# gpmp-dev/gpmp

Hardware: AMD Instinct MI355X
Metric: fp64 predict+NLL throughput (points/s) and potrf TFLOP/s vs roofline, n=32k (higher is better)
Workload: dtype f64

## Files before the change

gpmp_amd/_lib.py:

```python
from __future__ import annotations

import ctypes
import os
from ctypes import c_char_p, c_double, c_int, c_long, c_size_t, c_void_p

_HERE = os.path.dirname(os.path.abspath(__file__))
LIB_PATH = os.environ.get("GPMP_HIP_LIB") or os.path.join(_HERE, "libgpmp_hip.so")

_lib = None

_P = c_void_p
SIGNATURES = {
    "gpmp_hip_abi_version": (c_int, []),
    "gpmp_last_error": (c_char_p, []),
    "gpmp_profile_begin": (c_int, []),
    "gpmp_profile_begin_kinds": (c_int, [ctypes.c_uint]),
    "gpmp_profile_end": (c_int, [_P]),
    "gpmp_stream_create_reserving_cus": (c_int, [c_int, _P]),
    "gpmp_stream_destroy": (c_int, [_P]),
    "gpmp_stream_release": (c_int, [_P]),
    "gpmp_hint_machine_busy": (c_int, [c_int]),
    "gpmp_matern_gram": (c_int, [_P, _P, c_int, c_int, c_int, c_int, _P, c_int, c_double, c_int, _P, c_long, _P]),
    "gpmp_matern_pairwise": (c_int, [_P, _P, c_int, c_int, c_int, _P, c_int, _P, _P]),
    "gpmp_scaled_distance": (c_int, [_P, _P, c_int, c_int, c_int, _P, _P, c_long, _P]),
    "gpmp_maternp_kernel": (c_int, [_P, c_long, c_int, _P, _P]),
    "gpmp_matern_gram_deriv": (c_int, [_P, c_int, c_int, c_int, _P, c_int, c_int, _P, c_long, _P]),
    "gpmp_dinv_elems": (c_size_t, [c_int]),
    "gpmp_potrf_lower_async": (c_int, [_P, c_int, c_long, _P, _P, _P]),
    "gpmp_potrf_trsm_lower_async": (c_int, [_P, c_int, c_long, _P, _P, _P, c_int, c_long, _P]),
    "gpmp_trsm_lower": (c_int, [_P, c_int, c_long, _P, _P, c_int, c_long, c_int, _P, _P]),
    "gpmp_solve_status": (c_int, [_P, _P]),
    "gpmp_trsm_right_lower": (c_int, [_P, c_int, c_long, _P, _P, c_int, c_long, _P]),
    "gpmp_trtri_diag_blocks": (c_int, [_P, c_int, c_long, _P, _P]),
    "gpmp_trtri_lower": (c_int, [_P, c_int, c_long, _P, _P, c_long, _P]),
    "gpmp_lauum_lower": (c_int, [_P, c_int, c_long, _P, c_long, _P]),
    "gpmp_tril": (c_int, [_P, c_int, c_long, _P]),
    "gpmp_symmetrize_from_lower": (c_int, [_P, c_int, c_long, _P]),
    "gpmp_dgemm": (c_int, [c_int, c_int, c_int, c_int, c_int, c_double, _P, c_long, _P, c_long, c_double, _P, c_long, c_int, _P]),
    "gpmp_coldots": (c_int, [_P, c_int, c_int, c_long, _P, c_int, c_long, _P, c_long, _P, _P]),
    "gpmp_coldots_ws_rows": (c_int, [c_int]),
    "gpmp_device_release": (c_int, []),
    "gpmp_device_state_count": (c_int, []),
    "gpmp_debug_device_table_selftest": (c_int, [c_int, c_int, c_int]),
    "gpmp_jacobi_sweep": (c_int, [_P, c_long, _P, c_long, c_int, c_double, _P, _P]),
# ... 72 lines not shown
```

gpmp_amd/csrc/common.h:

```cpp
#pragma once
#include <hip/hip_runtime.h>
#include <cstdint>
#include <cstdio>
#include <cstring>
#include <atomic>
#include <vector>
#include "../../include/gpmp_hip.h"

namespace gpmp {

typedef double d4 __attribute__((ext_vector_type(4)));
typedef double d2 __attribute__((ext_vector_type(2)));

constexpr int NB = GPMP_NB;
constexpr int OUTER_BLOCKS = 4;

void set_error(const char* fmt, ...);
int hip_fail(hipError_t e, const char* what);

#define GPMP_HIP_TRY(expr)                                   \
  do {                                                       \
    hipError_t e__ = (expr);                                 \
    if (e__ != hipSuccess) return ::gpmp::hip_fail(e__, #expr); \
  } while (0)
// ... 40 lines not shown
};

struct GemmOpts {
  int lower_only = 0;
  int kstart_row = 0;
  int kend_row = 0;
  int kstart_col = 0;
  int kend_col = 0;
  int batch = 1;
  long stride_a = 0, stride_b = 0, stride_c = 0;
  int batch2 = 1;
  long stride2_a = 0, stride2_b = 0, stride2_c = 0;
  int lean = 0;
  int stair_num = 0, stair_den = 0, stair_off = 0, stair_sub = 0;
  int kg_rnum = 0, kg_rden = 0, kg_roff = 0, kg_cnum = 0, kg_cden = 0, kg_coff = 0;
};
int launch_gemm(bool a_kc, bool b_kc, int M, int N, int K, double alpha, const double* A, long lda,
                const double* B, long ldb, double beta, double* C, long ldc, const GemmOpts& o,
                hipStream_t st);

int launch_trsm_leaf_forward(const double* L, long ldl, const double* dinv_leaf, int nb, double* B, long ldb, int ncols,
                             double* G, hipStream_t st);

int launch_potf2_inv(double* A, long lda, int jb, double* dinv, int* info_dev, int offset, hipStream_t st);
int launch_potf2_inv_batch(double* A, long lda, int jb, double* dinv, int* info_dev, int offset, int nprob, long stride_a,
                           long stride_dinv, hipStream_t st);
int launch_trtri_blocks(const double* L, long ldl, int n, double* dinv, hipStream_t st);

constexpr int TRSV_FEW_MAX = 16;
int trsv_few(const double* L, int n, long ldl, const double* dinv, double* B, int m, long ldb, int trans,
             hipStream_t st);

int launch_tril(double* A, int n, long lda, hipStream_t st, int nprob = 1, long prob_stride = 0);
int launch_symmetrize(double* A, int n, long lda, hipStream_t st);
int launch_diag_blocks(double* T, int n, long ldt, const double* dinv, hipStream_t st, int nprob = 1, long prob_stride_t = 0,
                       long prob_stride_dinv = 0);

struct ProblemBatch {
  int nprob = 1;
  long stride_a = 0;
  long stride_dinv = 0;
};
int potrf_blocked_batch(double* A, int n, long lda, double* dinv, int* info_dev, const ProblemBatch& pb, hipStream_t st);
int trtri_doubling_batch(const double* L, int n, long ldl, const double* dinv, double* T, long ldt, const ProblemBatch& pb,
                         long stride_t, hipStream_t st);
int launch_gram_lower_batch(const double* x, long stride_x, const int* ns_dev, int nmax, int d, int p, const double* theta_host,
                            int noise, double diag_add, double* K, long ldk, long stride_k, int nprob, hipStream_t st,
                            const double* pp_dev = nullptr);
int gram_param_block_elems();
void fill_gram_param_block(double* blk, int d, int p, const double* theta, int noise, double diag_add);
int launch_grad_trace_batch(const double* Kinv, long ldk, long stride_kinv, const double* x, long stride_x, const int* ns_dev, int nmax,
// ... 7 lines not shown
```

gpmp_amd/csrc/drivers.hip:

```cpp
#include "matern_device.h"

namespace gpmp {
namespace {

constexpr int QMAX = GPMP_MAX_RANK - 1;
constexpr int QLD = QMAX + 1;

constexpr int SM_LDS = 0, SM_LDP = 1, SM_QUAD = 2, SM_ZKZ = 3, SM_C = 16, SM_TOTAL = 16 + QLD + 8;

__global__ void pack_zp_kernel(const double* __restrict__ z, const double* __restrict__ P, long ldp, int n, int q,
                               double* __restrict__ Y, long ldy) {
  const int i = blockIdx.x * blockDim.x + threadIdx.x;
  if (i >= n) return;
  Y[(long)i * ldy] = z[i];
  for (int a = 0; a < q; ++a) Y[(long)i * ldy + 1 + a] = P[(long)i * ldp + a];
}

__device__ int chol_lds(double (*A)[QLD + 1], int q, int* fail, double* d0) {
  const int t = threadIdx.x, nt = blockDim.x;
  for (int k = t; k < q; k += nt) d0[k] = A[k][k];
  for (int k = 0; k < q; ++k) {
    __syncthreads();
    if (t == 0) {
      const double dkk = A[k][k];
// ... 228 lines not shown


enum : unsigned {
  WS_T = 1u << 0,
  WS_W = 1u << 1,
  WS_X = 1u << 2,
  WS_FG = 1u << 3,
  WS_KIT = 1u << 4,
  WS_MEAN = 1u << 5,
  WS_SCAL = 1u << 6,
  WS_DCOL = 1u << 7,
  WS_PGRAD = 1u << 8,
};
struct DriverLayout {
  long ldn, ldm, ldq;
  size_t K, dinv, T, W, X, F, G, Kit, Gm, PtP, Sinv, small, scal, D, dcol, cd, y, vraw, mu, red, gws, total;
};
DriverLayout driver_layout(int n, int m, int d, int q, unsigned use) {
  DriverLayout l = {};
  l.ldn = pad16(n);
  l.ldm = pad16(m + 2 + q);
  l.ldq = pad16(1 + q);
  const size_t nq = (size_t)n * l.ldq, q1 = (size_t)(q > 0 ? q : 1);
  WsCursor c;
  l.K = c.take((size_t)n * l.ldn);
  l.dinv = c.take(gpmp_dinv_elems(n));
  if (use & WS_T) l.T = c.take((size_t)n * l.ldn);
  if (use & WS_W) l.W = c.take(nq);
  if (use & WS_X) l.X = c.take(nq);
  if (use & WS_FG) { l.F = c.take(nq); l.G = c.take(nq); }
  if (use & WS_KIT) l.Kit = c.take((size_t)n * l.ldm);
// ... 3 lines not shown
    l.Sinv = c.take(q1 * l.ldq);
    l.small = c.take(SM_TOTAL);
  }
  if (use & WS_SCAL) l.scal = c.take(16);
  if (use & WS_KIT) l.D = c.take((size_t)(2 + q) * l.ldm);
  if (use & WS_DCOL) l.dcol = c.take((size_t)n);
  const size_t cd_cols = (use & WS_DCOL) ? (size_t)n : (size_t)(m > 1 + q ? m : 1 + q);
  l.cd = c.take(cd_cols * (size_t)gpmp_coldots_ws_rows(n));
  if (use & WS_PGRAD) {
    l.y = c.take((size_t)n);
    l.vraw = c.take((size_t)m);
    l.mu = c.take(q1 * l.ldm);
    l.red = c.take(gpmp_predict_grad_reduce_ws_elems(n, m, d));
  }
  if (use & WS_FG) l.gws = c.take(gpmp_grad_ws_elems(n, d));
  l.total = c.at;
  return l;
}
constexpr unsigned USE_NLL = WS_W | WS_SCAL;
constexpr unsigned USE_REML = WS_W | WS_MEAN | WS_SCAL;
constexpr unsigned USE_NLL_GRAD = USE_REML | WS_T | WS_X | WS_FG;
constexpr unsigned USE_LOO = USE_REML | WS_T | WS_X | WS_DCOL;
constexpr unsigned USE_PREDICT = WS_KIT;
constexpr unsigned USE_PREDICT_MEAN = WS_KIT | WS_MEAN;
constexpr unsigned USE_PREDICT_GRAD = WS_KIT | WS_MEAN | WS_PGRAD;

struct Cov {
  const double* theta;
  int d, p, noise;
  double sigma2, diag;
// ... 80 lines not shown
}

int predict_solve(const Cov& cov, const DriverLayout& l, const double* xi, const double* zi, const double* Pi, long ldpi,
                  const double* xt, int n, int m, int q, double* ws, int* info_dev, gpmp_stream_t stream) {
  hipStream_t st = as_stream(stream);
  double* K = ws + l.K;
  double* Kit = ws + l.Kit;
  int rc = gpmp_matern_gram(xi, nullptr, n, n, cov.d, cov.p, cov.theta, cov.noise, cov.diag, 1, K, l.ldn, stream);
  if (rc) return rc;
  rc = gpmp_matern_gram(xi, xt, n, m, cov.d, cov.p, cov.theta, cov.noise, 0.0, 0, Kit, l.ldm, stream);
  if (rc) return rc;
  rc = stage_zp(zi, Pi, ldpi, n, q, Kit + m, l.ldm, st);
  if (rc) return rc;
  const int mb = (m + 1 + q) + ((m + 1 + q) & 1);
  if (mb > m + 1 + q) GPMP_HIP_TRY(hipMemset2DAsync(Kit + m + 1 + q, (size_t)l.ldm * sizeof(double), 0, sizeof(double), n, st));
  return gpmp_potrf_trsm_lower_async(K, n, l.ldn, ws + l.dinv, info_dev, Kit, mb, l.ldm, stream);
}
}
}

using namespace gpmp;

extern "C" size_t gpmp_nll_ws_elems(int n) { return n > 0 ? driver_layout(n, 0, 1, 0, USE_NLL).total : 0; }

extern "C" int gpmp_nll_zero_mean(const double* x, const double* z, int n, int d, int p, const double* theta_host,
                                  int noise, double* ws, double* nll_dev, int* info_dev, gpmp_stream_t stream) {
  GPMP_ARG(x != nullptr, 1, "x is NULL");
  GPMP_ARG(z != nullptr, 2, "z is NULL");
  GPMP_ARG(n > 0 && n <= GPMP_MAX_EXTENT, 3, "n outside [1, GPMP_MAX_EXTENT]");
  GPMP_ARG(theta_host != nullptr, 6, "theta is NULL");
  GPMP_ARG(ws != nullptr, 8, "ws is NULL");
// ... 243 lines not shown
```

gpmp_amd/csrc/gemm_f64.hip:

```cpp
#include "common.h"
#include <cstdlib>

namespace gpmp {

int g_machine_busy = 0;

namespace {

constexpr int BM = 128, BN = 128, BK = 16;
constexpr int LDK = 18;
constexpr int LDN = 144;
constexpr int TILE = 2304;
constexpr int NXCD = 8;
typedef unsigned int v4u __attribute__((ext_vector_type(4)));

struct GemmParams {
  const double* A;
  const double* B;
  double* C;
  long lda, ldb, ldc;
  int M, N, K;
  double alpha, beta;
  int lower_only, kstart_row, kend_row, kend_col;
  int kstart_col;
  int tiles_m, tiles_n, ntiles;
  int aligned;
  int lean;
  int batch;
  int batch2;
  int tri_block;
  int bn;
  int early;
  int stair_num, stair_den, stair_off, stair_sub;
  int kg_rnum, kg_rden, kg_roff, kg_cnum, kg_cden, kg_coff;
  long sa, sb, sc;
  long sa2, sb2, sc2;
};

__host__ __device__ __forceinline__ int stair_cols(int num, int den, int off, int sub, int tiles_n, int g) {
  const int a = num * g + off;
  if (a < 0) return 0;
  const int c = 8 * (a / den + 1 - sub);
  return c < 0 ? 0 : (c > tiles_n ? tiles_n : c);
}

__device__ __forceinline__ int group_kstart(const GemmParams& p, int ti, int tj) {
  int kb = 0;
  if (p.kg_rden > 0) {
    const int a = p.kg_rnum * (ti >> 3) + p.kg_roff;
    if (a > 0) kb = 1024 * ((a + p.kg_rden - 1) / p.kg_rden);
  }
// ... 320 lines not shown
constexpr int V2_TILE = 2048;

__device__ __forceinline__ double swap_lane_xor1(double v) {
  int lo = __double2loint(v), hi = __double2hiint(v);
  lo = __builtin_amdgcn_mov_dpp(lo, 0xB1, 0xF, 0xF, true);
  hi = __builtin_amdgcn_mov_dpp(hi, 0xB1, 0xF, 0xF, true);
  return __hiloint2double(hi, lo);
}

template <bool KC>
__device__ __forceinline__ int v2_frag_addr(int idx, int k) {
  if constexpr (KC) return idx * 16 + 2 * ((k >> 1) ^ ((idx >> 1) & 7)) + (k & 1);
  else return k * 128 + 2 * ((idx >> 1) ^ ((k & 1) << 3)) + (idx & 1);
}

template <bool AKC, bool BKC, bool CACC, int BNT = BN>
__global__ void __launch_bounds__(256, 2) gemm_f64_kernel_v2(GemmParams p) {
  constexpr int MI = BNT == BN ? 4 : 2;
  constexpr int NJ = BNT == BN ? 4 : BNT / 16;
  extern __shared__ __attribute__((aligned(16))) double smem[];
  int ti, tj;
  p.A += (long)blockIdx.y * p.sa + (long)blockIdx.z * p.sa2;
  p.B += (long)blockIdx.y * p.sb + (long)blockIdx.z * p.sb2;
  p.C += (long)blockIdx.y * p.sc + (long)blockIdx.z * p.sc2;
  decode_tile(p, blockIdx.x, ti, tj);
  ti = __builtin_amdgcn_readfirstlane(ti);
  tj = __builtin_amdgcn_readfirstlane(tj);
  const int row0 = ti * BM, col0 = tj * BNT;
  const int t = threadIdx.x;
  const int lane = t & 63;
  const int wave = __builtin_amdgcn_readfirstlane(t >> 6);
  const int wm = BNT == BN ? (wave >> 1) * 64 : wave * 32, wn = BNT == BN ? (wave & 1) * 64 : 0;
// ... 165 lines not shown
          v2u craw[4];
#pragma unroll
          for (int r = 0; r < 4; ++r)
            craw[r] = __builtin_amdgcn_raw_buffer_load_b64(rc, cvoff, (i * 16 + 4 * r) * ldc8 + j * 128, 0);
          ktile(T, true, [&] {
#pragma unroll
            for (int r = 0; r < 4; ++r) acc[i][j][r] = fma(sc, __builtin_bit_cast(double, craw[r]), acc[i][j][r]);
          });
        }
        kt = MI * NJ;
      }
    }
    for (; kt < nk; ++kt) ktile(kt, kt + 1 < nk, nothing);
  }

  if (!edge && (CACC || beta == 0.0)) {
    const bool odd = lane & 1;
    const unsigned off2 = lane_off - (odd ? 1u : 0u);
#pragma unroll
    for (int i = 0; i < MI; ++i)
#pragma unroll
      for (int j = 0; j < NJ; ++j) {
        const double a0 = alpha * acc[i][j][0], a1 = alpha * acc[i][j][1], a2 = alpha * acc[i][j][2], a3 = alpha * acc[i][j][3];
        const double g0 = swap_lane_xor1(odd ? a0 : a2), g1 = swap_lane_xor1(odd ? a1 : a3);
        const d2 v0 = odd ? (d2){g0, a2} : (d2){a0, g0};
        const d2 v1 = odd ? (d2){g1, a3} : (d2){a1, g1};
        double* rp0 = cbase + (long)(i * 16 + (odd ? 8 : 0)) * p.ldc + off2 + j * 16;
        *reinterpret_cast<d2*>(rp0) = v0;
        *reinterpret_cast<d2*>(rp0 + 4 * p.ldc) = v1;
      }
// ... 432 lines not shown
    else if (small_nt) {
      constexpr long below16 = 160;
      const long wg32 = (long)((p.N + SBN - 1) / SBN) * ((p.M + SBM - 1) / SBM);
      if (wg32 < below16) hipLaunchKernelGGL(gemm_nt_small_kernel<16>, dim3((p.N + SBN - 1) / SBN, (p.M + 15) / 16), dim3(256), 0, st, p);
      else hipLaunchKernelGGL(gemm_nt_small_kernel<SBM>, dim3((p.N + SBN - 1) / SBN, (p.M + SBM - 1) / SBM), dim3(256), 0, st, p);
    }
    else if (v2ok && pf.bn == 112) hipLaunchKernelGGL((gemm_f64_kernel_v2<AKC, BKC, CACC, 112>), dim3(pf.ntiles, pf.batch, pf.batch2), dim3(256), lds2, st, pf);
    else if (v2ok && pf.bn == 96) hipLaunchKernelGGL((gemm_f64_kernel_v2<AKC, BKC, CACC, 96>), dim3(pf.ntiles, pf.batch, pf.batch2), dim3(256), lds2, st, pf);
    else if (v2ok) hipLaunchKernelGGL((gemm_f64_kernel_v2<AKC, BKC, CACC>), dim3(p.ntiles, p.batch, p.batch2), dim3(256), lds2, st, p);
    else hipLaunchKernelGGL((gemm_f64_kernel<AKC, BKC, CACC>), dim3(p.ntiles, p.batch, p.batch2), dim3(256), lds, st, p);
  }
  GPMP_HIP_TRY(hipGetLastError());
  return 0;
}

template <bool AKC, bool BKC>
int launch_c(const GemmParams& p, hipStream_t st) {
  if (p.beta != 0.0 && p.alpha != 0.0) return launch_t<AKC, BKC, true>(p, st);
  return launch_t<AKC, BKC, false>(p, st);
}

}

int launch_trsm_leaf_forward(const double* L, long ldl, const double* dinv_leaf, int nb, double* B, long ldb, int ncols,
                             double* G, hipStream_t st) {
  if (ncols <= 0) return 0;
  const long ldg = (long)nb * BN;
  {
    LeafGParams g{L, ldl, dinv_leaf, G, ldg};
    hipLaunchKernelGGL(build_leaf_g_kernel, dim3(nb, nb), dim3(256), 0, st, g);
// ... 83 lines not shown
    const int tn = p.tiles_n < p.tiles_m ? p.tiles_n : p.tiles_m;
    p.ntiles = tn * (tn + 1) / 2 + (p.tiles_m - tn) * tn;
  } else {
    p.ntiles = p.tiles_m * p.tiles_n;
  }
  p.lean = o.lean | g_machine_busy;
  p.bn = BN;
  p.early = K >= 2048 ? 1 : 0;
  p.tri_block = !(o.kstart_row | o.kend_row | o.kstart_col | o.kend_col | o.kg_rden | o.kg_cden);
  p.batch = o.batch > 1 ? o.batch : 1;
  p.sa = o.stride_a; p.sb = o.stride_b; p.sc = o.stride_c;
  p.batch2 = o.batch2 > 1 ? o.batch2 : 1;
  p.sa2 = o.stride2_a; p.sb2 = o.stride2_b; p.sc2 = o.stride2_c;
  p.aligned = ((reinterpret_cast<uintptr_t>(A) & 15) == 0) && ((lda & 1) == 0) &&
              ((reinterpret_cast<uintptr_t>(B) & 15) == 0) && ((ldb & 1) == 0);
  if (a_kc && b_kc) return launch_c<true, true>(p, st);
  if (a_kc && !b_kc) return launch_c<true, false>(p, st);
  if (!a_kc && !b_kc) return launch_c<false, false>(p, st);
  return launch_c<false, true>(p, st);
}

int launch_gemm(bool a_kc, bool b_kc, int M, int N, int K, double alpha, const double* A, long lda,
                const double* B, long ldb, double beta, double* C, long ldc, const GemmOpts& o,
                hipStream_t st) {
  if (M <= 0 || N <= 0) return 0;
  const bool plain = !o.lower_only && !o.stair_den && !o.kg_rden && !o.kg_cden && !o.kstart_row && !o.kend_row && !o.kstart_col && !o.kend_col && o.batch <= 1 && o.batch2 <= 1;
  const int Nr = N % 2, Mr = M % 2;
  if (plain && (Nr || Mr) && (K % BK == 0) && K >= 512 && (M >= 4 * BM || N >= 4 * BN) && C != A && C != B) {
    const int Mf = M - Mr, Nf = N - Nr;
    int rc = 0;
    if (Mf > 0 && Nf > 0) rc = launch_gemm_one(a_kc, b_kc, Mf, Nf, K, alpha, A, lda, B, ldb, beta, C, ldc, o, st);
    if (rc) return rc;
    if (Nr > 0) {
      const double* Bn = b_kc ? B + (long)Nf * ldb : B + Nf;
      rc = launch_gemm_one(a_kc, b_kc, M, Nr, K, alpha, A, lda, Bn, ldb, beta, C + Nf, ldc, o, st);
      if (rc) return rc;
    }
    if (Mr > 0 && Nf > 0) {
      const double* Am = a_kc ? A + (long)Mf * lda : A + Mf;
      rc = launch_gemm_one(a_kc, b_kc, Mr, Nf, K, alpha, Am, lda, B, ldb, beta, C + (long)Mf * ldc, ldc, o, st);
    }
// ... 7 lines not shown
```

gpmp_amd/csrc/linalg.hip:

```cpp
#include "common.h"
#include <vector>
#include <cstdlib>
#include <mutex>
#include <map>
#include <memory>
#include <thread>
#include <atomic>

namespace gpmp {
namespace {

inline int imin(int a, int b) { return a < b ? a : b; }
inline int imax(int a, int b) { return a > b ? a : b; }

int potrf_blocked(double* A, int n, long lda, double* dinv, int* info_dev, int row0, hipStream_t st,
                  const ProblemBatch* pb = nullptr) {
  const int nblk = (n + NB - 1) / NB;
  GemmOpts lower;
  lower.lower_only = 1;
  GemmOpts plain;
  GemmOpts scale;
  if (pb != nullptr && pb->nprob > 1) {
    lower.batch2 = plain.batch2 = scale.batch2 = pb->nprob;
    lower.stride2_a = lower.stride2_b = lower.stride2_c = pb->stride_a;
// ... 209 lines not shown
    const int j = (s0 - p0) / sub;
    int W = sub;
    for (int t = j + 1; (t & 1) == 0; t >>= 1) W <<= 1;
    const int k0 = s1 - W;
    const int rest_cols = imin(imin(p1, n), s1 + W) - s1;
    if (rest_cols > 0 && k0 >= p0) {
      { int rcw = need_cols(s1 + rest_cols); if (rcw) return rcw; }
      int rc = launch_gemm(true, true, n - s1, rest_cols, s1 - k0, -1.0, A + (long)s1 * lda + k0, lda,
                           A + (long)s1 * lda + k0, lda, 1.0, A + (long)s1 * lda + s1, lda, lower, st);
      if (rc) return rc;
    }
  }
  return need_cols(p1 + 1);
}

int trsm_forward(const double* L, int n, long ldl, const double* dinv, double* B, int m, long ldb, double* gws, hipStream_t st);

struct SolveAlong {
  double* B = nullptr;
  int m = 0;
  long ldb = 0;
  double* gws = nullptr;
};

constexpr int LA_WIDE_ABOVE = 4096;
constexpr int LA_LEAN_ABOVE = 4096;
constexpr int LA_SPLIT_ABOVE = 8192;
constexpr int LA_MAIN_AFTER_LA_BELOW = 4096;

int potrf_lookahead(double* A, int n, long lda, double* dinv, int* info_dev, hipStream_t s0, const SolveAlong* sa = nullptr) {
  int dev = 0;
// ... 129 lines not shown
    hipEvent_t e_rows = g_la.next();
    GPMP_HIP_TRY(hipEventRecord(e_rows, g_solve_stream));
    GPMP_HIP_TRY(hipStreamWaitEvent(s0, e_rows, 0));
  }
  return 0;
}

constexpr int POTRF_ONE_STREAM_MAX = 4 * OUTER_BLOCKS * NB;

int potrf_lower(double* A, int n, long lda, double* dinv, int* info_dev, hipStream_t st) {
  GPMP_HIP_TRY(hipMemsetAsync(info_dev, 0, sizeof(int), st));
  if (n <= POTRF_ONE_STREAM_MAX) return potrf_blocked(A, n, lda, dinv, info_dev, 0, st);
  return potrf_lookahead(A, n, lda, dinv, info_dev, st);
}

int trsm_forward(const double* L, int n, long ldl, const double* dinv, double* B, int m, long ldb, double* gws, hipStream_t st) {
  if (n <= LEAF_TRSM) {
    const bool ok = gws != nullptr && n % NB == 0 && m >= 4 * NB && (m % 2 == 0) && (ldb % 2 == 0) &&
                    ((reinterpret_cast<uintptr_t>(B) & 15) == 0) && ((long)n * ldb * 8 < 0x7FFFFFFFL);
    if (ok) return launch_trsm_leaf_forward(L, ldl, dinv, n / NB, B, ldb, m, gws, st);
    return trsm_forward_blocked(L, n, ldl, dinv, B, m, ldb, st);
  }
  const int n1 = split_point(n);
  int rc = trsm_forward(L, n1, ldl, dinv, B, m, ldb, gws, st);
  if (rc) return rc;
  GemmOpts plain;
  rc = launch_gemm(true, false, n - n1, m, n1, -1.0, L + (long)n1 * ldl, ldl, B, ldb, 1.0, B + (long)n1 * ldb, ldb, plain, st);
  if (rc) return rc;
  return trsm_forward(L + (long)n1 * ldl + n1, n - n1, ldl, dinv + (size_t)(n1 / NB) * NB * NB, B + (long)n1 * ldb, m, ldb, gws, st);
}

int trsm_backward(const double* L, int n, long ldl, const double* dinv, double* B, int m, long ldb, hipStream_t st) {
  if (n <= LEAF_TRSM) return trsm_backward_blocked(L, n, ldl, dinv, B, m, ldb, st);
  const int n1 = split_point(n);
  int rc = trsm_backward(L + (long)n1 * ldl + n1, n - n1, ldl, dinv + (size_t)(n1 / NB) * NB * NB, B + (long)n1 * ldb, m,
                         ldb, st);
  if (rc) return rc;
  GemmOpts plain;
  rc = launch_gemm(false, false, n1, m, n - n1, -1.0, L + (long)n1 * ldl, ldl, B + (long)n1 * ldb, ldb, 1.0, B, ldb, plain, st);
  if (rc) return rc;
  return trsm_backward(L, n1, ldl, dinv, B, m, ldb, st);
}

int trtri_doubling(const double* L, int n, long ldl, const double* dinv, double* T, long ldt, hipStream_t st,
// ... 143 lines not shown
  if (n <= 0) return 0;
  return (size_t)((n + NB - 1) / NB) * NB * NB + (n > 2 * OUTER_BLOCKS * NB ? (size_t)4 * OUTER_BLOCKS * OUTER_BLOCKS * NB * NB : 0);
}

extern "C" int gpmp_potrf_lower_async(double* A, int n, long lda, double* dinv, int* info_dev,
                                      gpmp_stream_t stream) {
  GPMP_ARG(A != nullptr, 1, "A is NULL");
  GPMP_ARG(n >= 0 && n <= GPMP_MAX_EXTENT, 2, "n outside [0, GPMP_MAX_EXTENT]");
  GPMP_ARG(lda >= n, 3, "lda < n");
  GPMP_ARG(dinv != nullptr, 4, "dinv is NULL");
  GPMP_ARG(info_dev != nullptr, 5, "info is NULL");
  if (n == 0) return 0;
  return potrf_lower(A, n, lda, dinv, info_dev, as_stream(stream));
}

extern "C" int gpmp_potrf_trsm_lower_async(double* A, int n, long lda, double* dinv, int* info_dev, double* B, int m, long ldb,
                                           gpmp_stream_t stream) {
  GPMP_ARG(A != nullptr, 1, "A is NULL");
  GPMP_ARG(n >= 0 && n <= GPMP_MAX_EXTENT, 2, "n outside [0, GPMP_MAX_EXTENT]");
  GPMP_ARG(lda >= n, 3, "lda < n");
  GPMP_ARG(dinv != nullptr, 4, "dinv is NULL");
  GPMP_ARG(info_dev != nullptr, 5, "info_dev is NULL");
  GPMP_ARG(B != nullptr, 6, "B is NULL");
  GPMP_ARG(m >= 0 && m <= GPMP_MAX_EXTENT && ldb >= m, 8, "m outside [0, GPMP_MAX_EXTENT] or ldb < m");
  if (n == 0) return 0;
  hipStream_t st = as_stream(stream);
  GPMP_HIP_TRY(hipMemsetAsync(info_dev, 0, sizeof(int), st));
  double* gws = (n > 2 * OUTER_BLOCKS * NB) ? dinv + (size_t)((n + NB - 1) / NB) * NB * NB : nullptr;
  constexpr int along_above = 2 * OUTER_BLOCKS * NB, along_below = 8192;
  if (m > TRSV_FEW_MAX && n > along_above && n <= along_below) {
    SolveAlong sa;
    sa.B = B; sa.m = m; sa.ldb = ldb; sa.gws = gws;
    return potrf_lookahead(A, n, lda, dinv, info_dev, st, &sa);
  }
  int rc = (n <= POTRF_ONE_STREAM_MAX) ? potrf_blocked(A, n, lda, dinv, info_dev, 0, st) : potrf_lookahead(A, n, lda, dinv, info_dev, st);
  if (rc || m == 0) return rc;
  if (m <= TRSV_FEW_MAX) return trsv_few(A, n, lda, dinv, B, m, ldb, 0, st);
  return trsm_forward(A, n, lda, dinv, B, m, ldb, gws, st);
}

extern "C" int gpmp_trtri_diag_blocks(const double* L, int n, long ldl, double* dinv, gpmp_stream_t stream) {
  GPMP_ARG(L != nullptr, 1, "L is NULL");
  GPMP_ARG(n <= GPMP_MAX_EXTENT, 2, "n above GPMP_MAX_EXTENT");
  GPMP_ARG(ldl >= n, 3, "ldl < n");
  GPMP_ARG(dinv != nullptr, 4, "dinv is NULL");
  return launch_trtri_blocks(L, ldl, n, dinv, as_stream(stream));
}

extern "C" int gpmp_trsm_lower(const double* L, int n, long ldl, const double* dinv, double* B, int m,
                               long ldb, int trans, double* scratch, gpmp_stream_t stream) {
  GPMP_ARG(L != nullptr, 1, "L is NULL");
  GPMP_ARG(n >= 0 && n <= GPMP_MAX_EXTENT, 2, "n outside [0, GPMP_MAX_EXTENT]");
  GPMP_ARG(ldl >= n, 3, "ldl < n");
// ... 62 lines not shown
```

gpmp_amd/csrc/reduce.hip:

```cpp
#include "common.h"

namespace gpmp {
namespace {

constexpr int CD_R = 8;
constexpr int CD_MAX_CHUNKS = 32;

__global__ void __launch_bounds__(256) coldots_partial_kernel(const double* __restrict__ V, int n, int m,
                                                              long ldv, const double* __restrict__ Y,
                                                              int k0, int rk, long ldy, int rows_per,
                                                              int want_sq, double* __restrict__ partial) {
  const int j = blockIdx.x * 256 + threadIdx.x;
  const int chunk = blockIdx.y;
  const int i0 = chunk * rows_per;
  const int i1 = (i0 + rows_per) < n ? (i0 + rows_per) : n;
  double acc[CD_R];
#pragma unroll
  for (int k = 0; k < CD_R; ++k) acc[k] = 0.0;
  double sq = 0.0;
  if (j < m) {
#pragma unroll 4
    for (int i = i0; i < i1; ++i) {
      const double v = V[(long)i * ldv + j];
      const double* yr = Y + (long)i * ldy + k0;
// ... 93 lines not shown
}

__global__ void diag_blocks_kernel(double* __restrict__ T, int n, long ldt, const double* __restrict__ dinv, long prob_stride_t,
                                   long prob_stride_dinv) {
  T += (long)blockIdx.y * prob_stride_t;
  dinv += (long)blockIdx.y * prob_stride_dinv;
  const int b = blockIdx.x, b0 = b * NB;
  const int jb = (n - b0) < NB ? (n - b0) : NB;
  const double* D = dinv + (size_t)b * NB * NB;
  for (int idx = threadIdx.x; idx < NB * NB; idx += blockDim.x) {
    const int i = idx >> 7, j = idx & (NB - 1);
    if (i < jb && j < jb) T[(long)(b0 + i) * ldt + b0 + j] = D[idx];
  }
}

}

int launch_tril(double* A, int n, long lda, hipStream_t st, int nprob, long prob_stride) {
  if (n <= 1) return 0;
  hipLaunchKernelGGL(tril_kernel, dim3((n + 255) / 256, n < 16384 ? n : 16384, nprob), dim3(256), 0, st, A, n, lda, prob_stride);
  GPMP_HIP_TRY(hipGetLastError());
  return 0;
}
int launch_symmetrize(double* A, int n, long lda, hipStream_t st) {
  if (n <= 1) return 0;
  const int nb = (n + 31) / 32;
  hipLaunchKernelGGL(symmetrize_kernel, dim3(nb, nb), dim3(256), 0, st, A, n, lda);
  GPMP_HIP_TRY(hipGetLastError());
  return 0;
}
// ... 90 lines not shown
```

include/gpmp_hip.h:

```cpp
#ifndef GPMP_HIP_H
#define GPMP_HIP_H

#include <stddef.h>

#ifdef __cplusplus
extern "C" {
#endif

typedef void* gpmp_stream_t;

#define GPMP_NB 128
#define GPMP_MAX_DIM 64
#define GPMP_MAX_DIM_WIDE 16384
#define GPMP_MAX_P 16
#define GPMP_MAX_RANK 72
#define GPMP_MAX_EXTENT (1 << 30)
#define GPMP_BATCH_MAX_N 4096
#define GPMP_BATCH_MAX_Q 16

int gpmp_hip_abi_version(void);
const char* gpmp_last_error(void);

int gpmp_profile_begin(void);
int gpmp_profile_begin_kinds(unsigned kinds);
// ... 14 lines not shown
int gpmp_scaled_distance(const double* x, const double* y, int n, int m, int d,
                         const double* loginvrho_host, double* D, long ldd, gpmp_stream_t stream);

int gpmp_maternp_kernel(const double* h, long count, int p, double* out, gpmp_stream_t stream);

int gpmp_matern_gram_deriv(const double* x, int n, int d, int p, const double* theta_host, int noise,
                           int jparam, double* out, long ld, gpmp_stream_t stream);


size_t gpmp_dinv_elems(int n);

int gpmp_potrf_lower_async(double* A, int n, long lda, double* dinv, int* info_dev, gpmp_stream_t stream);

int gpmp_potrf_trsm_lower_async(double* A, int n, long lda, double* dinv, int* info_dev, double* B, int m, long ldb,
                                gpmp_stream_t stream);

int gpmp_trsm_lower(const double* L, int n, long ldl, const double* dinv, double* B, int m, long ldb,
                    int trans, double* scratch, gpmp_stream_t stream);

int gpmp_solve_status(gpmp_stream_t stream, int* status_host);
int gpmp_stream_release(gpmp_stream_t stream);
int gpmp_device_release(void);
int gpmp_device_state_count(void);
int gpmp_debug_device_table_selftest(int threads, int ordinals, int iters);

int gpmp_trsm_right_lower(const double* L, int k, long ldl, const double* dinv, double* B, int M, long ldb,
                          gpmp_stream_t stream);

int gpmp_trtri_diag_blocks(const double* L, int n, long ldl, double* dinv, gpmp_stream_t stream);

// ... 107 lines not shown
```

Before: 44730.

## Use one-level Strassen for large trailing updates in forward triangular solve

Large GEMM updates in the recursive forward TRSM (n1 >= 8192 rows, m >= 16384 right-hand sides) are replaced by a one-level Strassen scheme with seven half-size products instead of eight. A new GEMM epilogue mode writes each product into two destination blocks with separate signs, and a block-sum kernel builds the operand sums. Scratch space is reserved in the driver workspace for the Kit path, and the solve-along-potrf path is skipped when Strassen applies. This cuts arithmetic but adds memory passes for the sums and accumulations, and it slightly changes fp64 rounding behaviour.

```diff
diff --git a/gpmp_amd/_lib.py b/gpmp_amd/_lib.py
--- a/gpmp_amd/_lib.py
+++ b/gpmp_amd/_lib.py
@@ -28,6 +28,10 @@
     "gpmp_dinv_elems": (c_size_t, [c_int]),
     "gpmp_potrf_lower_async": (c_int, [_P, c_int, c_long, _P, _P, _P]),
     "gpmp_potrf_trsm_lower_async": (c_int, [_P, c_int, c_long, _P, _P, _P, c_int, c_long, _P]),
+    "gpmp_strassen_ws_elems": (c_size_t, [c_int, c_int]),
+    "gpmp_set_strassen_thresholds": (None, [c_int, c_int]),
+    "gpmp_debug_strassen_ws_elems": (c_size_t, [c_int, c_int]),
+    "gpmp_debug_strassen_update": (c_int, [_P, c_long, _P, c_long, _P, c_long, c_int, c_int, _P, c_size_t, _P]),
     "gpmp_trsm_lower": (c_int, [_P, c_int, c_long, _P, _P, c_int, c_long, c_int, _P, _P]),
     "gpmp_solve_status": (c_int, [_P, _P]),
     "gpmp_trsm_right_lower": (c_int, [_P, c_int, c_long, _P, _P, c_int, c_long, _P]),
diff --git a/gpmp_amd/csrc/common.h b/gpmp_amd/csrc/common.h
--- a/gpmp_amd/csrc/common.h
+++ b/gpmp_amd/csrc/common.h
@@ -78,6 +78,9 @@
   int lean = 0;
   int stair_num = 0, stair_den = 0, stair_off = 0, stair_sub = 0;
   int kg_rnum = 0, kg_rden = 0, kg_roff = 0, kg_cnum = 0, kg_cden = 0, kg_coff = 0;
+  double* c2 = nullptr;
+  long ldc2 = 0;
+  double sign1 = 1.0, sign2 = 1.0;
 };
 int launch_gemm(bool a_kc, bool b_kc, int M, int N, int K, double alpha, const double* A, long lda,
                 const double* B, long ldb, double beta, double* C, long ldc, const GemmOpts& o,
@@ -99,6 +102,11 @@
 int launch_symmetrize(double* A, int n, long lda, hipStream_t st);
 int launch_diag_blocks(double* T, int n, long ldt, const double* dinv, hipStream_t st, int nprob = 1, long prob_stride_t = 0,
                        long prob_stride_dinv = 0);
+int launch_block_sum(const double* X, long ldx, const double* Y, long ldy, double sign, double* D, long ldd, int rows, int cols,
+                     hipStream_t st);
+
+int potrf_trsm_lower_ws(double* A, int n, long lda, double* dinv, int* info_dev, double* B, int m, long ldb, double* sws,
+                        size_t sws_elems, hipStream_t st);
 
 struct ProblemBatch {
   int nprob = 1;
diff --git a/gpmp_amd/csrc/drivers.hip b/gpmp_amd/csrc/drivers.hip
--- a/gpmp_amd/csrc/drivers.hip
+++ b/gpmp_amd/csrc/drivers.hip
@@ -266,7 +266,7 @@
 };
 struct DriverLayout {
   long ldn, ldm, ldq;
-  size_t K, dinv, T, W, X, F, G, Kit, Gm, PtP, Sinv, small, scal, D, dcol, cd, y, vraw, mu, red, gws, total;
+  size_t K, dinv, T, W, X, F, G, Kit, Gm, PtP, Sinv, small, scal, D, dcol, cd, y, vraw, mu, red, gws, sws, sws_elems, total;
 };
 DriverLayout driver_layout(int n, int m, int d, int q, unsigned use) {
   DriverLayout l = {};
@@ -300,6 +300,10 @@
     l.red = c.take(gpmp_predict_grad_reduce_ws_elems(n, m, d));
   }
   if (use & WS_FG) l.gws = c.take(gpmp_grad_ws_elems(n, d));
+  if (use & WS_KIT) {
+    l.sws_elems = gpmp_strassen_ws_elems(n, (m + 1 + q) + ((m + 1 + q) & 1));
+    l.sws = c.take(l.sws_elems);
+  }
   l.total = c.at;
   return l;
 }
@@ -410,7 +414,7 @@
   if (rc) return rc;
   const int mb = (m + 1 + q) + ((m + 1 + q) & 1);
   if (mb > m + 1 + q) GPMP_HIP_TRY(hipMemset2DAsync(Kit + m + 1 + q, (size_t)l.ldm * sizeof(double), 0, sizeof(double), n, st));
-  return gpmp_potrf_trsm_lower_async(K, n, l.ldn, ws + l.dinv, info_dev, Kit, mb, l.ldm, stream);
+  return potrf_trsm_lower_ws(K, n, l.ldn, ws + l.dinv, info_dev, Kit, mb, l.ldm, l.sws_elems ? ws + l.sws : nullptr, l.sws_elems, st);
 }
 }
 }
diff --git a/gpmp_amd/csrc/gemm_f64.hip b/gpmp_amd/csrc/gemm_f64.hip
--- a/gpmp_amd/csrc/gemm_f64.hip
+++ b/gpmp_amd/csrc/gemm_f64.hip
@@ -35,6 +35,9 @@
   int kg_rnum, kg_rden, kg_roff, kg_cnum, kg_cden, kg_coff;
   long sa, sb, sc;
   long sa2, sb2, sc2;
+  double* C2;
+  long ldc2;
+  double sign1, sign2;
 };
 
 __host__ __device__ __forceinline__ int stair_cols(int num, int den, int off, int sub, int tiles_n, int g) {
@@ -385,8 +388,9 @@
   else return k * 128 + 2 * ((idx >> 1) ^ ((k & 1) << 3)) + (idx & 1);
 }
 
-template <bool AKC, bool BKC, bool CACC, int BNT = BN>
+template <bool AKC, bool BKC, bool CACC, int BNT = BN, bool DUAL = false>
 __global__ void __launch_bounds__(256, 2) gemm_f64_kernel_v2(GemmParams p) {
+  static_assert(!DUAL || !CACC, "the two-destination epilogue starts from zero accumulators");
   constexpr int MI = BNT == BN ? 4 : 2;
   constexpr int NJ = BNT == BN ? 4 : BNT / 16;
   extern __shared__ __attribute__((aligned(16))) double smem[];
@@ -582,6 +586,56 @@
     for (; kt < nk; ++kt) ktile(kt, kt + 1 < nk, nothing);
   }
 
+  if constexpr (DUAL) {
+    double* __restrict__ cbase2 = p.C2 + (long)row0 * p.ldc2 + col0;
+    const double s1 = p.sign1 * alpha, s2 = p.sign2 * alpha;
+    const unsigned lane_off2 = (unsigned)((wm + lk) * (int)p.ldc2 + wn + lr);
+    if (!edge) {
+      const bool odd = lane & 1;
+      const unsigned o1 = lane_off - (odd ? 1u : 0u), o2 = lane_off2 - (odd ? 1u : 0u);
+#pragma unroll
+      for (int i = 0; i < MI; ++i) {
+        double* r1 = cbase + (long)(i * 16 + (odd ? 8 : 0)) * p.ldc + o1;
+        double* r2 = cbase2 + (long)(i * 16 + (odd ? 8 : 0)) * p.ldc2 + o2;
+        d2 c1[NJ][2], c2[NJ][2];
+#pragma unroll
+        for (int j = 0; j < NJ; ++j) {
+          c1[j][0] = *reinterpret_cast<const d2*>(r1 + j * 16);
+          c1[j][1] = *reinterpret_cast<const d2*>(r1 + 4 * p.ldc + j * 16);
+          c2[j][0] = *reinterpret_cast<const d2*>(r2 + j * 16);
+          c2[j][1] = *reinterpret_cast<const d2*>(r2 + 4 * p.ldc2 + j * 16);
+        }
+#pragma unroll
+        for (int j = 0; j < NJ; ++j) {
+          const double a0 = acc[i][j][0], a1 = acc[i][j][1], a2 = acc[i][j][2], a3 = acc[i][j][3];
+          const double g0 = swap_lane_xor1(odd ? a0 : a2), g1 = swap_lane_xor1(odd ? a1 : a3);
+          const d2 v0 = odd ? (d2){g0, a2} : (d2){a0, g0};
+          const d2 v1 = odd ? (d2){g1, a3} : (d2){a1, g1};
+          *reinterpret_cast<d2*>(r1 + j * 16) = c1[j][0] + s1 * v0;
+          *reinterpret_cast<d2*>(r1 + 4 * p.ldc + j * 16) = c1[j][1] + s1 * v1;
+          *reinterpret_cast<d2*>(r2 + j * 16) = c2[j][0] + s2 * v0;
+          *reinterpret_cast<d2*>(r2 + 4 * p.ldc2 + j * 16) = c2[j][1] + s2 * v1;
+        }
+      }
+    } else {
+#pragma unroll
+      for (int i = 0; i < MI; ++i)
+#pragma unroll
+        for (int r = 0; r < 4; ++r) {
+          double* rp = cbase + (long)(i * 16 + 4 * r) * p.ldc;
+          double* rq = cbase2 + (long)(i * 16 + 4 * r) * p.ldc2;
+          const bool rok = wm + i * 16 + 4 * r + lk < rows_v;
+#pragma unroll
+          for (int j = 0; j < NJ; ++j) {
+            if (rok && wn + j * 16 + lr < cols_v) {
+              rp[lane_off + j * 16] += s1 * acc[i][j][r];
+              rq[lane_off2 + j * 16] += s2 * acc[i][j][r];
+            }
+          }
+        }
+    }
+    return;
+  }
   if (!edge && (CACC || beta == 0.0)) {
     const bool odd = lane & 1;
     const unsigned off2 = lane_off - (odd ? 1u : 0u);
@@ -1044,6 +1098,49 @@
   return 0;
 }
 
+int launch_dual(const GemmParams& p, hipStream_t st) {
+  static DeviceOnce attr_once;
+  const size_t lds2 = sizeof(double) * 4 * V2_TILE;
+  if (const long long dev_bit = attr_once.need()) {
+    if (dev_bit < 0) { set_error("hipGetDevice failed or device ordinal above 62"); return -1; }
+    GPMP_HIP_TRY(hipFuncSetAttribute(reinterpret_cast<const void*>(gemm_f64_kernel_v2<true, false, false, BN, true>),
+                                     hipFuncAttributeMaxDynamicSharedMemorySize, (int)lds2));
+    GPMP_HIP_TRY(hipFuncSetAttribute(reinterpret_cast<const void*>(gemm_f64_kernel_v2<true, false, false, 112, true>),
+                                     hipFuncAttributeMaxDynamicSharedMemorySize, (int)lds2));
+    GPMP_HIP_TRY(hipFuncSetAttribute(reinterpret_cast<const void*>(gemm_f64_kernel_v2<true, false, false, 96, true>),
+                                     hipFuncAttributeMaxDynamicSharedMemorySize, (int)lds2));
+    attr_once.done(dev_bit);
+  }
+  const bool ok = p.aligned && (p.M % 2 == 0) && (p.N % 2 == 0) && (p.K % BK == 0) && p.K > 0 && p.alpha != 0.0 && p.beta == 1.0 &&
+                  ((reinterpret_cast<uintptr_t>(p.C) & 15) == 0) && (p.ldc % 2 == 0) && (p.ldc >= p.N) &&
+                  ((reinterpret_cast<uintptr_t>(p.C2) & 15) == 0) && (p.ldc2 % 2 == 0) && (p.ldc2 >= p.N) &&
+                  ((long)BM * p.lda * 8 + (long)p.K * 8 < 0x7FFFFFFFL) && ((long)BN * p.ldb * 8 + (long)p.K * 8 < 0x7FFFFFFFL) &&
+                  ((long)BM * p.ldc * 8 < 0x7FFFFFFFL) && ((long)BM * p.ldc2 * 8 < 0x7FFFFFFFL) &&
+                  p.batch == 1 && p.batch2 == 1 && !p.lower_only && !p.stair_den &&
+                  !(p.kstart_row | p.kend_row | p.kstart_col | p.kend_col | p.kg_rden | p.kg_cden);
+  if (!ok) { set_error("two-destination product: operands not 16-byte aligned, odd sizes, K not a multiple of 16, beta != 1 or a restricted tile set"); return -1; }
+  GemmParams pf = p;
+  if (p.N >= 16 * BN) {
+    const long slots = 2L * device_cu_count();
+    auto cost = [&](int w) { const long t = (long)p.tiles_m * ((p.N + w - 1) / w); return ((t + slots - 1) / slots) * (long)w; };
+    long best = cost(BN);
+    for (int w : {112, 96}) {
+      const long c = cost(w);
+      if (c * 100 < best * 97) { best = c; pf.bn = w; }
+    }
+    pf.tiles_n = (p.N + pf.bn - 1) / pf.bn;
+    pf.ntiles = pf.tiles_m * pf.tiles_n;
+  }
+  {
+    ProfScope ps(PK_GEMM2_NN, st, 2.0 * (double)p.M * (double)p.N * (double)p.K);
+    if (pf.bn == 112) hipLaunchKernelGGL((gemm_f64_kernel_v2<true, false, false, 112, true>), dim3(pf.ntiles), dim3(256), lds2, st, pf);
+    else if (pf.bn == 96) hipLaunchKernelGGL((gemm_f64_kernel_v2<true, false, false, 96, true>), dim3(pf.ntiles), dim3(256), lds2, st, pf);
+    else hipLaunchKernelGGL((gemm_f64_kernel_v2<true, false, false, BN, true>), dim3(pf.ntiles), dim3(256), lds2, st, pf);
+  }
+  GPMP_HIP_TRY(hipGetLastError());
+  return 0;
+}
+
 template <bool AKC, bool BKC>
 int launch_c(const GemmParams& p, hipStream_t st) {
   if (p.beta != 0.0 && p.alpha != 0.0) return launch_t<AKC, BKC, true>(p, st);
@@ -1157,6 +1254,11 @@
   p.sa2 = o.stride2_a; p.sb2 = o.stride2_b; p.sc2 = o.stride2_c;
   p.aligned = ((reinterpret_cast<uintptr_t>(A) & 15) == 0) && ((lda & 1) == 0) &&
               ((reinterpret_cast<uintptr_t>(B) & 15) == 0) && ((ldb & 1) == 0);
+  p.C2 = o.c2; p.ldc2 = o.ldc2; p.sign1 = o.sign1; p.sign2 = o.sign2;
+  if (o.c2 != nullptr) {
+    if (!(a_kc && !b_kc)) { set_error("two-destination product: NN kind only"); return -1; }
+    return launch_dual(p, st);
+  }
   if (a_kc && b_kc) return launch_c<true, true>(p, st);
   if (a_kc && !b_kc) return launch_c<true, false>(p, st);
   if (!a_kc && !b_kc) return launch_c<false, false>(p, st);
@@ -1167,7 +1269,7 @@
                 const double* B, long ldb, double beta, double* C, long ldc, const GemmOpts& o,
                 hipStream_t st) {
   if (M <= 0 || N <= 0) return 0;
-  const bool plain = !o.lower_only && !o.stair_den && !o.kg_rden && !o.kg_cden && !o.kstart_row && !o.kend_row && !o.kstart_col && !o.kend_col && o.batch <= 1 && o.batch2 <= 1;
+  const bool plain = !o.lower_only && !o.stair_den && !o.kg_rden && !o.kg_cden && !o.kstart_row && !o.kend_row && !o.kstart_col && !o.kend_col && o.batch <= 1 && o.batch2 <= 1 && o.c2 == nullptr;
   const int Nr = N % 2, Mr = M % 2;
   if (plain && (Nr || Mr) && (K % BK == 0) && K >= 512 && (M >= 4 * BM || N >= 4 * BN) && C != A && C != B) {
     const int Mf = M - Mr, Nf = N - Nr;
diff --git a/gpmp_amd/csrc/linalg.hip b/gpmp_amd/csrc/linalg.hip
--- a/gpmp_amd/csrc/linalg.hip
+++ b/gpmp_amd/csrc/linalg.hip
@@ -247,7 +247,9 @@
   return need_cols(p1 + 1);
 }
 
-int trsm_forward(const double* L, int n, long ldl, const double* dinv, double* B, int m, long ldb, double* gws, hipStream_t st);
+struct StrassenWs;
+int trsm_forward(const double* L, int n, long ldl, const double* dinv, double* B, int m, long ldb, double* gws, hipStream_t st,
+                 const StrassenWs* sw = nullptr);
 
 struct SolveAlong {
   double* B = nullptr;
@@ -407,7 +409,74 @@
   return potrf_lookahead(A, n, lda, dinv, info_dev, st);
 }
 
-int trsm_forward(const double* L, int n, long ldl, const double* dinv, double* B, int m, long ldb, double* gws, hipStream_t st) {
+constexpr int STRASSEN_MIN_ROWS = 8192;
+constexpr int STRASSEN_MIN_COLS = 16384;
+std::mutex g_strassen_mu;
+int g_strassen_min_rows = STRASSEN_MIN_ROWS, g_strassen_min_cols = STRASSEN_MIN_COLS;
+struct StrassenLimits { int rows, cols; };
+StrassenLimits strassen_limits() {
+  std::lock_guard<std::mutex> lk(g_strassen_mu);
+  return {g_strassen_min_rows, g_strassen_min_cols};
+}
+struct StrassenWs {
+  double* p = nullptr;
+  size_t elems = 0;
+  StrassenLimits lim = {STRASSEN_MIN_ROWS, STRASSEN_MIN_COLS};
+};
+
+inline int strassen_col_split(int N) { return (N / 2) / NB * NB; }
+inline bool strassen_shape_ok(int M, int K, int N) {
+  return M > 0 && K > 0 && M % (2 * NB) == 0 && K % (2 * NB) == 0 && N % 2 == 0 && strassen_col_split(N) >= NB;
+}
+inline size_t strassen_node_elems(int M, int K, int N) {
+  return (size_t)pad16((long)(M / 2) * (K / 2)) + (size_t)pad16((long)(K / 2) * strassen_col_split(N));
+}
+size_t strassen_solve_elems(int n, int m, const StrassenLimits& lim) {
+  if (n <= LEAF_TRSM) return 0;
+  const int n1 = split_point(n);
+  size_t need = (n1 >= lim.rows && m >= lim.cols && strassen_shape_ok(n - n1, n1, m)) ? strassen_node_elems(n - n1, n1, m) : 0;
+  const size_t a = strassen_solve_elems(n1, m, lim), b = strassen_solve_elems(n - n1, m, lim);
+  if (a > need) need = a;
+  if (b > need) need = b;
+  return need;
+}
+
+int strassen_update(const double* A, long lda, const double* B, long ldb, double* C, long ldc, int M, int K, int N, double* ws,
+                    hipStream_t st) {
+  const int Mh = M / 2, Kh = K / 2, Nh = strassen_col_split(N), Np = N - 2 * Nh;
+  const double *A11 = A, *A12 = A + Kh, *A21 = A + (long)Mh * lda, *A22 = A21 + Kh;
+  const double *B11 = B, *B12 = B + Nh, *B21 = B + (long)Kh * ldb, *B22 = B21 + Nh;
+  double *C11 = C, *C12 = C + Nh, *C21 = C + (long)Mh * ldc, *C22 = C21 + Nh;
+  double* S = ws;
+  double* T = ws + pad16((long)Mh * Kh);
+  auto lsum = [&](const double* X, const double* Y, double sign) { return launch_block_sum(X, lda, Y, lda, sign, S, Kh, Mh, Kh, st); };
+  auto rsum = [&](const double* X, const double* Y, double sign) { return launch_block_sum(X, ldb, Y, ldb, sign, T, Nh, Kh, Nh, st); };
+  auto prod = [&](const double* Ao, long ldao, const double* Bo, long ldbo, double* Ca, double sa, double* Cb, double sb) {
+    GemmOpts o;
+    o.c2 = Cb; o.ldc2 = ldc; o.sign1 = sa; o.sign2 = sb;
+    return launch_gemm(true, false, Mh, Nh, Kh, -1.0, Ao, ldao, Bo, ldbo, 1.0, Ca, ldc, o, st);
+  };
+  int rc;
+  if ((rc = lsum(A11, A22, 1.0)) || (rc = rsum(B11, B22, 1.0)) || (rc = prod(S, Kh, T, Nh, C11, 1.0, C22, 1.0))) return rc;
+  if ((rc = lsum(A21, A22, 1.0)) || (rc = prod(S, Kh, B11, ldb, C21, 1.0, C22, -1.0))) return rc;
+  if ((rc = rsum(B12, B22, -1.0)) || (rc = prod(A11, lda, T, Nh, C12, 1.0, C22, 1.0))) return rc;
+  if ((rc = rsum(B21, B11, -1.0)) || (rc = prod(A22, lda, T, Nh, C11, 1.0, C21, 1.0))) return rc;
+  if ((rc = lsum(A11, A12, 1.0)) || (rc = prod(S, Kh, B22, ldb, C11, -1.0, C12, 1.0))) return rc;
+  if ((rc = lsum(A21, A11, -1.0)) || (rc = rsum(B11, B12, 1.0)) || (rc = prod(S, Kh, T, Nh, C22, 1.0, nullptr, 0.0))) return rc;
+  if ((rc = lsum(A12, A22, -1.0)) || (rc = rsum(B21, B22, 1.0)) || (rc = prod(S, Kh, T, Nh, C11, 1.0, nullptr, 0.0))) return rc;
+  if (Np > 0) {
+    GemmOpts plain;
+    rc = launch_gemm(true, false, M, Np, K, -1.0, A, lda, B + 2 * Nh, ldb, 1.0, C + 2 * Nh, ldc, plain, st);
+  }
+  return rc;
+}
+
+inline bool strassen_operands_ok(const double* A, long lda, const double* B, long ldb) {
+  return ((reinterpret_cast<uintptr_t>(A) | reinterpret_cast<uintptr_t>(B)) & 15) == 0 && lda % 2 == 0 && ldb % 2 == 0;
+}
+
+int trsm_forward(const double* L, int n, long ldl, const double* dinv, double* B, int m, long ldb, double* gws, hipStream_t st,
+                 const StrassenWs* sw) {
   if (n <= LEAF_TRSM) {
     const bool ok = gws != nullptr && n % NB == 0 && m >= 4 * NB && (m % 2 == 0) && (ldb % 2 == 0) &&
                     ((reinterpret_cast<uintptr_t>(B) & 15) == 0) && ((long)n * ldb * 8 < 0x7FFFFFFFL);
@@ -415,12 +484,18 @@
     return trsm_forward_blocked(L, n, ldl, dinv, B, m, ldb, st);
   }
   const int n1 = split_point(n);
-  int rc = trsm_forward(L, n1, ldl, dinv, B, m, ldb, gws, st);
+  int rc = trsm_forward(L, n1, ldl, dinv, B, m, ldb, gws, st, sw);
   if (rc) return rc;
-  GemmOpts plain;
-  rc = launch_gemm(true, false, n - n1, m, n1, -1.0, L + (long)n1 * ldl, ldl, B, ldb, 1.0, B + (long)n1 * ldb, ldb, plain, st);
+  const double* L21 = L + (long)n1 * ldl;
+  if (sw != nullptr && sw->p != nullptr && n1 >= sw->lim.rows && m >= sw->lim.cols && strassen_shape_ok(n - n1, n1, m) &&
+      strassen_operands_ok(L21, ldl, B, ldb) && sw->elems >= strassen_node_elems(n - n1, n1, m)) {
+    rc = strassen_update(L21, ldl, B, ldb, B + (long)n1 * ldb, ldb, n - n1, n1, m, sw->p, st);
+  } else {
+    GemmOpts plain;
+    rc = launch_gemm(true, false, n - n1, m, n1, -1.0, L21, ldl, B, ldb, 1.0, B + (long)n1 * ldb, ldb, plain, st);
+  }
   if (rc) return rc;
-  return trsm_forward(L + (long)n1 * ldl + n1, n - n1, ldl, dinv + (size_t)(n1 / NB) * NB * NB, B + (long)n1 * ldb, m, ldb, gws, st);
+  return trsm_forward(L + (long)n1 * ldl + n1, n - n1, ldl, dinv + (size_t)(n1 / NB) * NB * NB, B + (long)n1 * ldb, m, ldb, gws, st, sw);
 }
 
 int trsm_backward(const double* L, int n, long ldl, const double* dinv, double* B, int m, long ldb, hipStream_t st) {
@@ -594,8 +669,44 @@
   return potrf_lower(A, n, lda, dinv, info_dev, as_stream(stream));
 }
 
+extern "C" size_t gpmp_strassen_ws_elems(int n, int m) {
+  if (n <= 0 || m <= TRSV_FEW_MAX || n > GPMP_MAX_EXTENT || m > GPMP_MAX_EXTENT) return 0;
+  return strassen_solve_elems(n, m, strassen_limits());
+}
+
+extern "C" void gpmp_set_strassen_thresholds(int min_rows, int min_cols) {
+  std::lock_guard<std::mutex> lk(g_strassen_mu);
+  g_strassen_min_rows = min_rows > 0 ? min_rows : STRASSEN_MIN_ROWS;
+  g_strassen_min_cols = min_cols > 0 ? min_cols : STRASSEN_MIN_COLS;
+}
+
+extern "C" size_t gpmp_debug_strassen_ws_elems(int R, int N) {
+  return (R > 0 && N > 0 && R <= GPMP_MAX_EXTENT && N <= GPMP_MAX_EXTENT && strassen_shape_ok(R, R, N)) ? strassen_node_elems(R, R, N) : 0;
+}
+
+extern "C" int gpmp_debug_strassen_update(const double* L21, long ldl, const double* X1, long ldx, double* B2, long ldb, int R, int N,
+                                          double* scratch, size_t scratch_elems, gpmp_stream_t stream) {
+  GPMP_ARG(L21 != nullptr, 1, "L21 is NULL");
+  GPMP_ARG(X1 != nullptr, 3, "X1 is NULL");
+  GPMP_ARG(B2 != nullptr, 5, "B2 is NULL");
+  GPMP_ARG(R > 0 && R <= GPMP_MAX_EXTENT && R % (2 * NB) == 0, 7, "R outside [256, GPMP_MAX_EXTENT] or not a multiple of 256");
+  GPMP_ARG(N >= 2 * NB && N <= GPMP_MAX_EXTENT && N % 2 == 0, 8, "N outside [256, GPMP_MAX_EXTENT] or odd");
+  GPMP_ARG(ldl >= R && ldl % 2 == 0, 2, "ldl < R or odd");
+  GPMP_ARG(ldx >= N && ldx % 2 == 0, 4, "ldx < N or odd");
+  GPMP_ARG(ldb >= N && ldb % 2 == 0, 6, "ldb < N or odd");
+  GPMP_ARG(scratch != nullptr && scratch_elems >= strassen_node_elems(R, R, N), 9, "scratch is NULL or below gpmp_debug_strassen_ws_elems");
+  GPMP_ARG(((reinterpret_cast<uintptr_t>(L21) | reinterpret_cast<uintptr_t>(X1) | reinterpret_cast<uintptr_t>(B2) |
+             reinterpret_cast<uintptr_t>(scratch)) & 15) == 0, 1, "an operand is not 16-byte aligned");
+  return strassen_update(L21, ldl, X1, ldx, B2, ldb, R, R, N, scratch, as_stream(stream));
+}
+
 extern "C" int gpmp_potrf_trsm_lower_async(double* A, int n, long lda, double* dinv, int* info_dev, double* B, int m, long ldb,
                                            gpmp_stream_t stream) {
+  return potrf_trsm_lower_ws(A, n, lda, dinv, info_dev, B, m, ldb, nullptr, 0, as_stream(stream));
+}
+
+int gpmp::potrf_trsm_lower_ws(double* A, int n, long lda, double* dinv, int* info_dev, double* B, int m, long ldb, double* sws,
+                              size_t sws_elems, hipStream_t st) {
   GPMP_ARG(A != nullptr, 1, "A is NULL");
   GPMP_ARG(n >= 0 && n <= GPMP_MAX_EXTENT, 2, "n outside [0, GPMP_MAX_EXTENT]");
   GPMP_ARG(lda >= n, 3, "lda < n");
@@ -604,11 +715,15 @@
   GPMP_ARG(B != nullptr, 6, "B is NULL");
   GPMP_ARG(m >= 0 && m <= GPMP_MAX_EXTENT && ldb >= m, 8, "m outside [0, GPMP_MAX_EXTENT] or ldb < m");
   if (n == 0) return 0;
-  hipStream_t st = as_stream(stream);
+  StrassenWs sw;
+  sw.lim = strassen_limits();
+  const size_t sneed = (sws != nullptr && m > TRSV_FEW_MAX) ? strassen_solve_elems(n, m, sw.lim) : 0;
+  GPMP_ARG(sws_elems >= sneed, 10, "Strassen scratch below gpmp_strassen_ws_elems(n, m)");
+  if (sneed > 0) { sw.p = sws; sw.elems = sws_elems; }
   GPMP_HIP_TRY(hipMemsetAsync(info_dev, 0, sizeof(int), st));
   double* gws = (n > 2 * OUTER_BLOCKS * NB) ? dinv + (size_t)((n + NB - 1) / NB) * NB * NB : nullptr;
   constexpr int along_above = 2 * OUTER_BLOCKS * NB, along_below = 8192;
-  if (m > TRSV_FEW_MAX && n > along_above && n <= along_below) {
+  if (sneed == 0 && m > TRSV_FEW_MAX && n > along_above && n <= along_below) {
     SolveAlong sa;
     sa.B = B; sa.m = m; sa.ldb = ldb; sa.gws = gws;
     return potrf_lookahead(A, n, lda, dinv, info_dev, st, &sa);
@@ -616,7 +731,7 @@
   int rc = (n <= POTRF_ONE_STREAM_MAX) ? potrf_blocked(A, n, lda, dinv, info_dev, 0, st) : potrf_lookahead(A, n, lda, dinv, info_dev, st);
   if (rc || m == 0) return rc;
   if (m <= TRSV_FEW_MAX) return trsv_few(A, n, lda, dinv, B, m, ldb, 0, st);
-  return trsm_forward(A, n, lda, dinv, B, m, ldb, gws, st);
+  return trsm_forward(A, n, lda, dinv, B, m, ldb, gws, st, sneed > 0 ? &sw : nullptr);
 }
 
 extern "C" int gpmp_trtri_diag_blocks(const double* L, int n, long ldl, double* dinv, gpmp_stream_t stream) {
diff --git a/gpmp_amd/csrc/reduce.hip b/gpmp_amd/csrc/reduce.hip
--- a/gpmp_amd/csrc/reduce.hip
+++ b/gpmp_amd/csrc/reduce.hip
@@ -131,6 +131,42 @@
   }
 }
 
+__global__ void __launch_bounds__(256) block_sum_kernel(const double* __restrict__ X, long ldx, const double* __restrict__ Y, long ldy,
+                                                        double sign, double* __restrict__ D, long ldd, int rows, int pairs) {
+  for (int c = blockIdx.x * 256 + threadIdx.x; c < pairs; c += gridDim.x * 256) {
+    int r = blockIdx.y;
+    for (; r + 3 * (int)gridDim.y < rows; r += 4 * gridDim.y) {
+      d2 x[4], y[4];
+#pragma unroll
+      for (int u = 0; u < 4; ++u) {
+        const long rr = r + u * (long)gridDim.y;
+        x[u] = *reinterpret_cast<const d2*>(X + rr * ldx + 2 * c);
+        y[u] = *reinterpret_cast<const d2*>(Y + rr * ldy + 2 * c);
+      }
+#pragma unroll
+      for (int u = 0; u < 4; ++u) *reinterpret_cast<d2*>(D + (r + u * (long)gridDim.y) * ldd + 2 * c) = x[u] + sign * y[u];
+    }
+    for (; r < rows; r += gridDim.y)
+      *reinterpret_cast<d2*>(D + (long)r * ldd + 2 * c) =
+          *reinterpret_cast<const d2*>(X + (long)r * ldx + 2 * c) + sign * *reinterpret_cast<const d2*>(Y + (long)r * ldy + 2 * c);
+  }
+}
+
+}
+
+int launch_block_sum(const double* X, long ldx, const double* Y, long ldy, double sign, double* D, long ldd, int rows, int cols,
+                     hipStream_t st) {
+  if (rows <= 0 || cols <= 0) return 0;
+  const bool ok = (cols % 2 == 0) && (ldx % 2 == 0) && (ldy % 2 == 0) && (ldd % 2 == 0) && ldx >= cols && ldy >= cols && ldd >= cols &&
+                  ((reinterpret_cast<uintptr_t>(X) | reinterpret_cast<uintptr_t>(Y) | reinterpret_cast<uintptr_t>(D)) & 15) == 0;
+  if (!ok) { set_error("block sum: odd column count or leading dimension, or an operand not 16-byte aligned"); return -1; }
+  const int pairs = cols / 2;
+  const int gx = (pairs + 255) / 256 < 64 ? (pairs + 255) / 256 : 64;
+  int gy = (16 * device_cu_count() + gx - 1) / gx;
+  if (gy > (rows + 3) / 4) gy = (rows + 3) / 4;
+  hipLaunchKernelGGL(block_sum_kernel, dim3(gx, gy), dim3(256), 0, st, X, ldx, Y, ldy, sign, D, ldd, rows, pairs);
+  GPMP_HIP_TRY(hipGetLastError());
+  return 0;
 }
 
 int launch_tril(double* A, int n, long lda, hipStream_t st, int nprob, long prob_stride) {
diff --git a/include/gpmp_hip.h b/include/gpmp_hip.h
--- a/include/gpmp_hip.h
+++ b/include/gpmp_hip.h
@@ -52,6 +52,12 @@
 
 int gpmp_potrf_trsm_lower_async(double* A, int n, long lda, double* dinv, int* info_dev, double* B, int m, long ldb,
                                 gpmp_stream_t stream);
+
+size_t gpmp_strassen_ws_elems(int n, int m);
+void gpmp_set_strassen_thresholds(int min_rows, int min_cols);
+size_t gpmp_debug_strassen_ws_elems(int R, int N);
+int gpmp_debug_strassen_update(const double* L21, long ldl, const double* X1, long ldx, double* B2, long ldb, int R, int N,
+                               double* scratch, size_t scratch_elems, gpmp_stream_t stream);
 
 int gpmp_trsm_lower(const double* L, int n, long ldl, const double* dinv, double* B, int m, long ldb,
                     int trans, double* scratch, gpmp_stream_t stream);
```

Result: faster. 46340, median of 6 (+3.6%).
